# bcgsc/abyss

Hardware: NVIDIA B200
Metric: k-mers/sec (Bloom insert + unitig extend) (higher is better)
Workload: dtype u8

## Files before the change

### abyss_b200/capi.py

```python
from __future__ import annotations

import ctypes as C
import os

import numpy as np

_HERE = os.path.dirname(os.path.abspath(__file__))
LIB_PATH = os.path.join(_HERE, "lib", "libabyssb200.so")

ABB_OK, ABB_EINVAL, ABB_ENODEV, ABB_ECUDA, ABB_ENOMEM, ABB_ESTATE = 0, -1, -2, -3, -4, -5
COUNTING, BIT, CASCADING = 0, 1, 2


class AbbError(RuntimeError):
    def __init__(self, code: int, msg: str):
        super().__init__(f"libabyssb200 error {code}: {msg}")
        self.code = code


class InsertStats(C.Structure):
    _fields_ = [("kmers", C.c_uint64), ("slots", C.c_uint64), ("windows", C.c_uint64),
                ("deferred", C.c_uint64), ("launches", C.c_uint64),
                ("ms_hash", C.c_float), ("ms_insert", C.c_float), ("ms_commit", C.c_float),
                ("commit_launches", C.c_uint64), ("commit_slots", C.c_uint64), ("drains", C.c_uint64),
# ... 60 lines not shown
    "abb_filter_set_threshold": (C.c_int, [_vp, C.c_uint]),
    "abb_insert_reads": (C.c_int, [_vp, _vp, _vp, C.c_uint64, _u64p]),
    "abb_insert_reads_dev": (C.c_int, [_vp, _vp, _vp, C.c_uint64, C.c_uint64, _u64p]),
    "abb_insert_hashes": (C.c_int, [_vp, _vp, C.c_uint64]),
    "abb_contains_hashes": (C.c_int, [_vp, _vp, C.c_uint64, _vp]),
    "abb_mincount_hashes": (C.c_int, [_vp, _vp, C.c_uint64, _vp]),
    "abb_hash_reads": (C.c_int, [C.c_uint, C.c_char_p, _vp, _vp, C.c_uint64, _vp, _vp, _u64p, C.c_int]),
    "abb_hash_reads_dev": (C.c_int, [_vp, _vp, _vp, C.c_uint64, _vp, _vp, C.c_uint64, _u64p]),
    "abb_insert_h0_dev": (C.c_int, [_vp, _vp, C.c_uint64]),
    "abb_comm_unique_id": (C.c_int, [_vp]),
    "abb_comm_create": (C.c_int, [C.POINTER(_vp), C.c_int, C.c_int, _vp, C.c_int]),
    "abb_comm_destroy": (C.c_int, [_vp]),
    "abb_comm_rank": (C.c_int, [_vp]),
    "abb_comm_world": (C.c_int, [_vp]),
    "abb_insert_reads_sharded_dev": (C.c_int, [_vp, _vp, _vp, _vp, C.c_uint64, C.c_int, _u64p]),
    "abb_insert_reads_sharded": (C.c_int, [_vp, _vp, _vp, _vp, C.c_uint64, C.c_int, _u64p]),
    "abb_filter_resident_reads": (C.c_int, [_vp, C.POINTER(_vp), C.POINTER(_vp), _u64p]),
    "abb_filter_allgather": (C.c_int, [_vp, _vp]),
    "abb_comm_allgather_bytes": (C.c_int, [_vp, _vp, C.c_uint64, _vp]),
    "abb_comm_allreduce_max_u8": (C.c_int, [_vp, _vp, C.c_uint64, _vp]),
    "abb_comm_exchange_bytes": (C.c_int, [_vp, _vp, C.c_uint64, _vp, _u64p, _u64p, _vp]),
    "abb_filter_device_ptr": (_vp, [_vp, C.c_int]),
    "abb_filter_download": (C.c_int, [_vp, C.c_int, _vp, C.c_uint64]),
    "abb_filter_upload": (C.c_int, [_vp, C.c_int, _vp, C.c_uint64]),
    "abb_filter_clear": (C.c_int, [_vp]),
    "abb_filter_popcount": (C.c_int, [_vp, _u64p, _u64p]),
    "abb_assembler_create": (C.c_int, [C.POINTER(_vp), _vp, C.POINTER(AssemblyParams)]),
    "abb_assembler_destroy": (C.c_int, [_vp]),
    "abb_assembler_process_reads": (C.c_int, [_vp, _vp, _vp, C.c_uint64, C.POINTER(C.POINTER(Contig)), _u64p, C.POINTER(C.c_char_p)]),
    "abb_assembler_process_reads_dev": (C.c_int, [_vp, _vp, _vp, C.c_uint64, C.POINTER(C.POINTER(Contig)), _u64p, C.POINTER(C.c_char_p)]),
    "abb_assembler_stats": (C.c_int, [_vp, C.POINTER(AssemblyStats)]),
    "abb_assembler_reset": (C.c_int, [_vp]),
    "abb_assembler_classify_dev": (C.c_int, [_vp, _vp, _vp, C.c_uint64, _vp]),
    "abb_assembler_set_codes": (C.c_int, [_vp, _vp, C.c_uint64]),
    "abb_assembler_counters": (C.c_int, [_vp, C.POINTER(AssemblyCounters)]),
    "abb_assembler_set_counters": (C.c_int, [_vp, C.POINTER(AssemblyCounters)]),
    "abb_assembler_read_results": (C.c_int, [_vp, C.POINTER(_u8p), _u64p]),
    "abb_assembler_set_comm": (C.c_int, [_vp, _vp]),
    "abb_assembler_trace": (C.c_int, [_vp, C.POINTER(C.POINTER(TraceRow)), _u64p]),
    "abb_assembler_assembled_filter": (_vp, [_vp]),
    "abb_filter_insert_stats": (C.c_int, [_vp, C.POINTER(InsertStats), C.c_int]),
    "abb_filter_set_window": (C.c_int, [_vp, C.c_uint64]),
    "abb_filter_set_profiling": (C.c_int, [_vp, C.c_int]),
    "abb_filter_stream": (_vp, [_vp]),
    "abb_contains_reads": (C.c_int, [_vp, _vp, _vp, C.c_uint64, _vp, _vp, C.c_uint64, _u64p]),
    "abb_successors": (C.c_int, [_vp, _vp, C.c_uint64, C.c_uint, _vp, _vp, _vp]),
# ... 193 lines not shown
        h, n = self._hashes(hashes)
        out = np.zeros(n, dtype=np.uint8)
        check(self._lib.abb_contains_hashes(self._h, _ptr(h), n, _ptr(out)))
        return out.astype(bool)

    def minCount(self, hashes) -> np.ndarray:
        h, n = self._hashes(hashes)
        out = np.zeros(n, dtype=np.uint8)
        check(self._lib.abb_mincount_hashes(self._h, _ptr(h), n, _ptr(out)))
        return out

    def download(self, level: int = -1) -> np.ndarray:
        out = np.empty(self.sizeInBytes(), dtype=np.uint8)
        check(self._lib.abb_filter_download(self._h, level, _ptr(out), out.size))
        return out

    def upload(self, data: np.ndarray, level: int = -1):
        d = np.ascontiguousarray(data, dtype=np.uint8)
        check(self._lib.abb_filter_upload(self._h, level, _ptr(d), d.size))

    def clear(self):
        check(self._lib.abb_filter_clear(self._h))

    def popcounts(self) -> tuple[int, int]:
        a, b = C.c_uint64(0), C.c_uint64(0)
        check(self._lib.abb_filter_popcount(self._h, C.byref(a), C.byref(b)))
        return a.value, b.value

    def popCount(self): return self.popcounts()[0]
    def filtered_popcount(self): return self.popcounts()[1]
    def FPR(self): return (self.popCount() / self.size()) ** self.getHashNum()
    def filtered_FPR(self): return (self.filtered_popcount() / self.size()) ** self.getHashNum()

    def stats(self, reset: bool = False) -> InsertStats:
        st = InsertStats()
        check(self._lib.abb_filter_insert_stats(self._h, C.byref(st), int(reset)))
        return st


READ_CODES = ["SHORTER_THAN_K", "NON_ACGT", "BLUNT_END", "NOT_SOLID", "ALL_KMERS_VISITED", "GENERATED_CONTIGS", "CANDIDATE"]


class Assembler:

    def __init__(self, solid: Filter, trim: int | None = None, read_log: bool = False, verbose: int = 0):
        self._lib = load()
# ... 164 lines not shown
```

### abyss_b200/csrc/abb_api.cu

```cuda
#include "abb_common.h"
#include "abb_insert.cuh"
#include "abb_shard.cuh"
#include <dlfcn.h>
#include <nccl.h>
#include <cub/device/device_scan.cuh>
#include <algorithm>
#include <cstdlib>
#include <cstring>
#include <new>
#include <vector>

namespace abb {

static thread_local char g_err[512] = "";

void set_error(const char* fmt, ...)
{
	va_list ap;
	va_start(ap, fmt);
	vsnprintf(g_err, sizeof g_err, fmt, ap);
	va_end(ap);
}

constexpr uint64_t kDefaultWindow = 1ULL << 17;
// ... 18 lines not shown
	}
	if (device < 0 || device >= n) {
		set_error("device %d out of range (0..%d)", device, n - 1);
		return ABB_EINVAL;
	}
	ABB_CUDA(cudaSetDevice(device));
	static int fetch = -1;
	if (fetch < 0) {
		const char* e = getenv("ABB_L2_FETCH");
		fetch = e ? atoi(e) : 0;
	}
	if (fetch > 0)
		cudaDeviceSetLimit(cudaLimitMaxL2FetchGranularity, (size_t)fetch);
	return ABB_OK;
}

static FilterView view_of(const abb_filter* f)
{
	FilterView v;
	v.data = f->d_data;
	v.level_stride = f->bytes_per_level;
	v.levels = f->levels;
	return v;
}

static uint64_t map_entries_for(uint64_t filter_size, unsigned lg = 25)
{
	if (const char* e = getenv("ABB_MAP_LOG2")) {
		const int v = atoi(e);
		if (v >= 10 && v <= 32)
			lg = (unsigned)v;
	}
	uint64_t want = 1ULL << lg;
	const uint64_t fit = std::max<uint64_t>(next_pow2(filter_size), 1024);
	return std::min(want, fit);
}

static unsigned age_windows_for(uint64_t window)
{
	return (unsigned)std::min<uint64_t>(kMaxAgeWindows, ((1ULL << kPrioBits) - 2) / window - 1);
}

static int ensure_workspace(abb_filter* f)
{
	const uint64_t want_entries = map_entries_for(f->size, f->map_log2 ? f->map_log2 : 25);
	if (f->d_carry && f->ws_window == f->window && f->ws_H == f->H && f->map_entries == want_entries)
// ... 101 lines not shown
};

template <int KIND, bool LITERAL, int MAXH>
static int launch_windows(const InsertArgs& args, int device, cudaStream_t st)
{
	static int grid_cache[64] = { 0 };
	int& grid = grid_cache[device & 63];
	if (grid == 0) {
		int per_sm = 0, sms = 0;
		ABB_CUDA(cudaOccupancyMaxActiveBlocksPerMultiprocessor(&per_sm, k_insert_windows<KIND, LITERAL, MAXH>, 256, 0));
		ABB_CUDA(cudaDeviceGetAttribute(&sms, cudaDevAttrMultiProcessorCount, device));
		grid = std::max(1, per_sm) * sms;
	}
	void* params[] = { (void*)&args };
	ABB_CUDA(cudaLaunchCooperativeKernel((void*)k_insert_windows<KIND, LITERAL, MAXH>, dim3((unsigned)grid), dim3(256), params, 0, st));
	return ABB_OK;
}

template <bool LITERAL>
static int ordered_insert(abb_filter* f, const uint64_t* d_hashes, const uint8_t* d_valid, uint64_t n_slots)
{
	if (n_slots == 0)
		return ABB_OK;
	if (f->kind == ABB_BIT) {
		ABB_DISPATCH_H(f->H, (k_bits_insert<LITERAL, MAXH><<<blocks_for(n_slots, 256), 256, 0, f->stream>>>(
		                         d_hashes, d_valid, n_slots, f->cfg, f->d_data)));
		f->st.launches += 1;
		ABB_CUDA(cudaGetLastError());
		return ABB_OK;
	}
	ABB_CHECK(ensure_workspace(f));
	cudaStream_t st = f->stream;
	const uint64_t W = f->window;
	const uint64_t n_windows = (n_slots + W - 1) / W;
	ABB_REQUIRE(n_windows < (1ULL << 31), "too many windows in one call");
	const uint64_t cap = W + kCarryLanes;
	InsertArgs a;
	a.hashes = d_hashes;
	a.valid = d_valid;
	a.n_slots = n_slots;
	a.window = (unsigned)W;
	a.w_begin = 0;
	a.n_windows = (unsigned)n_windows;
	a.cfg = f->cfg;
	for (int i = 0; i < 3; ++i) {
		a.map[i].w = f->d_map[i];
// ... 332 lines not shown
}

struct abb_comm {
	ncclComm_t comm = nullptr;
	int rank = 0, world = 1, device = 0;
};

namespace abb {

static uint64_t shard_chunk(uint64_t size, unsigned world) { return ((size + world - 1) / world + 15) & ~15ULL; }

static uint64_t sharded_window(const abb_filter* f, unsigned world)
{
	uint64_t w = 2 * f->window * world;
	if (const char* e = getenv("ABB_SHARD_WINDOW"))
		w = strtoull(e, nullptr, 10);
	return std::min<uint64_t>(std::max<uint64_t>(w, 32), 1ULL << 21);
}

static int sharded_ordered_insert(abb_filter* f, abb_comm* c, const uint64_t* d_h0, const uint8_t* d_valid, uint64_t n_slots)
{
	if (n_slots == 0)
		return ABB_OK;
	const uint64_t user_window = f->window;
	f->window = sharded_window(f, (unsigned)c->world);
	f->map_log2 = 27;
	int rc = ensure_workspace(f);
	const uint64_t W = f->window;
	f->window = user_window;
	f->map_log2 = 0;
	ABB_CHECK(rc);
	const unsigned max_lanes = (unsigned)std::min<uint64_t>((uint64_t)kCarryLanes * (unsigned)c->world, W / 2 + kCarryLanes);
	ABB_CHECK(f->sh_buf.reserve(2 * (W + (uint64_t)max_lanes) + 64));
	cudaStream_t st = f->stream;
	const uint64_t n_windows = (n_slots + W - 1) / W;
	const unsigned age_off = (unsigned)(age_windows_for(W) * W);
	const unsigned drain_age = age_off / 3 * 2;
	const uint64_t cap = 3 * (W + kCarryLanes) / 2;
	uint64_t* carry[2] = { f->d_carry, f->d_carry + cap };
	ShardCtl* ctl = reinterpret_cast<ShardCtl*>(f->d_ctl);
	unsigned* d_nout = f->d_ctl + 4;
	const size_t map_bytes = std::max<size_t>(f->map_entries / 4, 256);
	ConflictMap maps[2] = { { f->d_map[0], f->map_entries - 1 }, { f->d_map[1], f->map_entries - 1 } };
	const uint64_t chunk = shard_chunk(f->size, (unsigned)c->world);
	Shard sh;
	sh.lo = std::min<uint64_t>(f->size, (uint64_t)c->rank * chunk);
// ... 193 lines not shown
	ABB_TRY(cudaMalloc((void**)&f->d_stats, 8 * sizeof(unsigned long long)));
	ABB_TRY(cudaMemsetAsync(f->d_stats, 0, 8 * sizeof(unsigned long long), f->stream));
	if (!f->mask.empty()) {
		std::vector<uint8_t> care(k);
		for (unsigned i = 0; i < k; ++i)
			care[i] = f->mask[i] == '1';
		ABB_TRY(cudaMalloc((void**)&f->d_care, k));
		ABB_TRY(cudaMemcpyAsync(f->d_care, care.data(), k, cudaMemcpyHostToDevice, f->stream));
	}
	ABB_TRY(cudaStreamSynchronize(f->stream));
#undef ABB_TRY
	*out = f;
	return ABB_OK;
}

int abb_filter_destroy(abb_filter* f)
{
	if (!f)
		return ABB_OK;
	cudaSetDevice(f->device);
	if (f->stream)
		cudaStreamSynchronize(f->stream);
	cudaFree(f->d_data);
	cudaFree(f->d_care);
	cudaFree(f->d_tags2[0]);
	cudaFree(f->d_tags2[1]);
	cudaFree(f->d_map[0]);
	cudaFree(f->d_carry);
	cudaFree(f->d_slotbits);
	cudaFree(f->d_ctl);
	cudaFree(f->d_stats);
	f->bases.release();
	f->offs.release();
	f->slot_offs.release();
	f->h0.release();
	f->lit.release();
	f->bounds.release();
	f->gq_kmers.release();
	f->gq_info.release();
	f->gq_len.release();
	f->gq_self.release();
	f->valid.release();
	f->scan_tmp.release();
	f->out8.release();
	f->sh_buf.release();
	for (auto e : f->prof_ev)
// ... 257 lines not shown
int abb_comm_destroy(abb_comm* c)
{
	if (!c)
		return ABB_OK;
	cudaSetDevice(c->device);
	if (c->comm && g_nccl.CommDestroy)
		g_nccl.CommDestroy(c->comm);
	delete c;
	return ABB_OK;
}

int abb_comm_rank(const abb_comm* c) { return c ? c->rank : 0; }
int abb_comm_world(const abb_comm* c) { return c ? c->world : 1; }

int abb_filter_allgather(abb_filter* f, abb_comm* c)
{
	ABB_REQUIRE(f && c, "NULL argument");
	ABB_REQUIRE(f->levels == 1, "only single-level filters are sharded");
	ABB_CUDA(cudaSetDevice(f->device));
	if (c->world == 1 || f->replicated_insert)
		return ABB_OK;
	const uint64_t chunk = shard_chunk(f->bytes_per_level, (unsigned)c->world);
	ABB_REQUIRE(chunk * c->world <= f->bytes_per_level + 4096, "too many ranks for the all-gather slack");
	ABB_NCCL(g_nccl.AllGather(f->d_data + (uint64_t)c->rank * chunk, f->d_data, chunk, ncclUint8, c->comm, f->stream));
	ABB_CUDA(cudaStreamSynchronize(f->stream));
	return ABB_OK;
}

int abb_comm_allgather_bytes(abb_comm* c, void* d_buf, uint64_t bytes_per_rank, void* cuda_stream)
{
	ABB_REQUIRE(c && (d_buf || bytes_per_rank == 0), "NULL argument");
	if (c->world == 1 || bytes_per_rank == 0)
		return ABB_OK;
	ABB_CUDA(cudaSetDevice(c->device));
	ABB_NCCL(g_nccl.AllGather((const uint8_t*)d_buf + (uint64_t)c->rank * bytes_per_rank, d_buf, bytes_per_rank, ncclUint8, c->comm,
	                          (cudaStream_t)cuda_stream));
	return ABB_OK;
}

int abb_comm_exchange_bytes(abb_comm* c, const void* d_send, uint64_t send_bytes, void* d_recv_base, const uint64_t* recv_offsets,
                            const uint64_t* recv_bytes, void* cuda_stream)
{
	ABB_REQUIRE(c && recv_offsets && recv_bytes, "NULL argument");
	if (c->world == 1)
		return ABB_OK;
	ABB_CUDA(cudaSetDevice(c->device));
// ... 27 lines not shown
	ABB_REQUIRE(f && c, "NULL argument");
	ABB_REQUIRE(f->kind == ABB_COUNTING, "the sharded insert is implemented for counting filters");
	ABB_REQUIRE(n_reads == 0 || (d_bases && d_offsets), "NULL read buffers");
	ABB_REQUIRE(f->device == c->device, "filter and communicator live on different devices");
	ABB_CUDA(cudaSetDevice(f->device));
	const bool shard = shard_policy(c->world);
	f->replicated_insert = !shard;
	ABB_CHECK(insert_reads_dev(f, (const uint8_t*)d_bases, d_offsets, n_reads, n_kmers_out, shard ? c : nullptr));
	if (finalize)
		ABB_CHECK(abb_filter_allgather(f, c));
	return ABB_OK;
}

void* abb_filter_device_ptr(abb_filter* f, int level)
{
	if (!f)
		return nullptr;
	if (level < 0)
		level = (int)f->levels - 1;
	if ((unsigned)level >= f->levels)
		return nullptr;
	cudaSetDevice(f->device);
	cudaStreamSynchronize(f->stream);
	return f->d_data + (uint64_t)level * f->bytes_per_level;
}

static int query_hashes(abb_filter* f, const uint64_t* hashes, uint64_t n, uint8_t* out, bool want_min)
{
	ABB_REQUIRE(f, "NULL filter");
	if (n == 0)
		return ABB_OK;
	ABB_REQUIRE(hashes && out, "NULL buffer");
	ABB_CUDA(cudaSetDevice(f->device));
	ABB_CHECK(f->lit.reserve(n * f->H));
	ABB_CHECK(f->out8.reserve(n));
	ABB_CUDA(cudaMemcpyAsync(f->lit.p, hashes, n * f->H * sizeof(uint64_t), cudaMemcpyHostToDevice, f->stream));
	const FilterView fv = view_of(f);
	if (f->kind == ABB_COUNTING)
		k_query<0><<<blocks_for(n, 256), 256, 0, f->stream>>>(f->lit.p, n, f->cfg, fv, f->threshold, want_min ? nullptr : f->out8.p,
		                                                       want_min ? f->out8.p : nullptr);
	else
		k_query<1><<<blocks_for(n, 256), 256, 0, f->stream>>>(f->lit.p, n, f->cfg, fv, 0, want_min ? nullptr : f->out8.p,
		                                                       want_min ? f->out8.p : nullptr);
	f->st.launches += 1;
	ABB_CUDA(cudaGetLastError());
	ABB_CUDA(cudaMemcpyAsync(out, f->out8.p, n, cudaMemcpyDeviceToHost, f->stream));
// ... 170 lines not shown
	ABB_REQUIRE(nbytes == f->bytes_per_level, "buffer is %llu bytes, the filter level is %llu", (unsigned long long)nbytes,
	            (unsigned long long)f->bytes_per_level);
	*p = f->d_data + (uint64_t)level * f->bytes_per_level;
	return ABB_OK;
}

int abb_filter_download(abb_filter* f, int level, uint8_t* host, uint64_t nbytes)
{
	uint8_t* p = nullptr;
	ABB_CHECK(level_ptr(f, level, nbytes, &p));
	ABB_REQUIRE(host, "NULL buffer");
	ABB_CUDA(cudaSetDevice(f->device));
	ABB_CUDA(cudaMemcpyAsync(host, p, nbytes, cudaMemcpyDeviceToHost, f->stream));
	ABB_CUDA(cudaStreamSynchronize(f->stream));
	return ABB_OK;
}

int abb_filter_upload(abb_filter* f, int level, const uint8_t* host, uint64_t nbytes)
{
	uint8_t* p = nullptr;
	ABB_CHECK(level_ptr(f, level, nbytes, &p));
	ABB_REQUIRE(host, "NULL buffer");
	ABB_CUDA(cudaSetDevice(f->device));
	ABB_CUDA(cudaMemcpyAsync(p, host, nbytes, cudaMemcpyHostToDevice, f->stream));
	ABB_CUDA(cudaStreamSynchronize(f->stream));
	return ABB_OK;
}

int abb_filter_clear(abb_filter* f)
{
	ABB_REQUIRE(f, "NULL filter");
	ABB_CUDA(cudaSetDevice(f->device));
	ABB_CUDA(cudaMemsetAsync(f->d_data, 0, f->bytes_per_level * f->levels, f->stream));
	ABB_CUDA(cudaStreamSynchronize(f->stream));
	return ABB_OK;
}

int abb_filter_popcount(abb_filter* f, uint64_t* nonzero, uint64_t* at_or_above_threshold)
{
	ABB_REQUIRE(f, "NULL filter");
	ABB_CUDA(cudaSetDevice(f->device));
	ABB_CUDA(cudaMemsetAsync(f->d_stats + 4, 0, 2 * sizeof(unsigned long long), f->stream));
	const uint8_t* p = f->d_data + (uint64_t)(f->levels - 1) * f->bytes_per_level;
	k_popcount<<<148 * 8, 256, 0, f->stream>>>(p, f->bytes_per_level, f->kind == ABB_COUNTING, f->threshold, f->d_stats + 4);
	f->st.launches += 1;
	ABB_CUDA(cudaGetLastError());
	unsigned long long h[2] = { 0, 0 };
	ABB_CUDA(cudaMemcpyAsync(h, f->d_stats + 4, sizeof h, cudaMemcpyDeviceToHost, f->stream));
	ABB_CUDA(cudaStreamSynchronize(f->stream));
	if (nonzero)
		*nonzero = h[0];
	if (at_or_above_threshold)
		*at_or_above_threshold = f->kind == ABB_COUNTING ? h[1] : h[0];
	return ABB_OK;
}

// ... 24 lines not shown
```

### abyss_b200/csrc/abb_assemble.cu

```cuda
#include "abb_common.h"
#include "abb_walk.cuh"
#include <cooperative_groups.h>
#include <cub/device/device_select.cuh>
#include <thrust/iterator/counting_iterator.h>
#include <algorithm>
#include <chrono>
#include <cstdlib>
#include <cstring>
#include <new>
#include <vector>

namespace abb {
namespace cg = cooperative_groups;

__host__ __device__ inline uint64_t tile_slot(uint64_t key, unsigned cls, unsigned mask)
{
	return (((key ^ (0x9E3779B97F4A7C15ULL * (cls + 1))) * 0xD6E8FEB86659FD93ULL) >> 24) & mask;
}

struct WarpCtx {
	unsigned k, trim;
	RollTab rt;
	const HashCfg* cfg;
	const uint8_t* counters;
	unsigned threshold;
	unsigned lane;
	Frame* frames;
	uint64_t* look;
	uint8_t* arena;
	unsigned long long arena_size;
	unsigned long long* arena_top;
	unsigned fail_;
	const TileRec* tile_recs;
	const unsigned* tile_tab;
	unsigned tile_mask;

	unsigned long long* dbg = nullptr;
	long long t_last = 0;
	__device__ void tick(int slot)
	{
		if (!dbg)
			return;
		const long long now = clock64();
		if (slot >= 0 && lane == 0)
			dbg[slot] += (unsigned long long)(now - t_last);
		t_last = now;
	}
	__device__ bool tiles_enabled() const { return tile_tab != nullptr; }
// ... 5 lines not shown
				return nullptr;
			const TileRec* t = tile_recs + (v - 1);
			if (t->key == key && t->cls == cls)
				return t;
		}
	}
	__device__ uint32_t tile_index(const TileRec* t) const { return (uint32_t)(t - tile_recs); }
	__device__ const TileRec* tile_at(uint32_t idx) const { return tile_recs + idx; }
	__device__ void prefetch(const void* p) const
	{
		if (p)
			asm volatile("prefetch.global.L2 [%0];" ::"l"(p));
	}
	__device__ void wr32(uint32_t* p, uint32_t v) const { *(volatile uint32_t*)p = v; }

	struct Probe {
		bool ok;
	};
	template <int KW>
	__device__ Probe neighbors_issue(const Vtx<KW>& v) const
	{
		const unsigned n = lane >> 2, hs = lane & 3;
		const uint64_t h0 = neighbor_bloom(v, k, rt, n < 4 ? FWD : REV, n & 3);
		unsigned mn = 255;
		for (unsigned i = hs; i < cfg->H; i += 4)
			mn = min(mn, (unsigned)__ldcg(counters + nth_pos(h0, *cfg, i)));
		Probe p;
		p.ok = mn >= threshold;
		return p;
	}
	__device__ unsigned neighbors_finish(const Probe& p) const
	{
		unsigned b = __ballot_sync(0xffffffffu, p.ok);
		b &= b >> 1;
		b &= b >> 2;
		unsigned r = 0;
#pragma unroll
		for (int j = 0; j < 8; ++j)
			r |= ((b >> (4 * j)) & 1u) << j;
		return r;
	}
	template <int KW>
	__device__ unsigned neighbors(const Vtx<KW>& v) const
	{
		return neighbors_finish(neighbors_issue(v));
	}
	template <int KW>
	__device__ unsigned neighbors_dir(const Vtx<KW>& v, Dir d) const
	{
		const unsigned n = lane >> 2, hs = lane & 3;
		const bool mine = (n < 4) == (d == FWD);
		bool ok = true;
		if (mine) {
			const uint64_t h0 = neighbor_bloom(v, k, rt, n < 4 ? FWD : REV, n & 3);
			unsigned mn = 255;
			for (unsigned i = hs; i < cfg->H; i += 4)
				mn = min(mn, (unsigned)__ldcg(counters + nth_pos(h0, *cfg, i)));
			ok = mn >= threshold;
		}
		Probe p;
		p.ok = ok;
		const unsigned m = neighbors_finish(p);
		return d == FWD ? (m & 15) : (m >> 4);
	}
	__device__ uint64_t rd64(const uint64_t* p) const { return *(const volatile uint64_t*)p; }
	__device__ void wr64(uint64_t* p, uint64_t v) const { *(volatile uint64_t*)p = v; }
	__device__ uint8_t rd8(const uint8_t* p) const { return *(const volatile uint8_t*)p; }
	__device__ void wr8(uint8_t* p, uint8_t v) const { *(volatile uint8_t*)p = v; }
	__device__ void sync() const { __syncwarp(); }
	__device__ bool find64(const uint64_t* a, unsigned n, uint64_t key, unsigned stride) const
	{
		for (unsigned base = 0; base < n; base += 32) {
			const unsigned i = base + lane;
			const bool hit = i < n && *(const volatile uint64_t*)(a + (size_t)i * stride) == key;
			if (__any_sync(0xffffffffu, hit))
				return true;
		}
		return false;
	}
	__device__ uint8_t* alloc(unsigned long long bytes, bool zero)
	{
// ... 242 lines not shown
				r.seed_pos = seed_pos;
				r.psize = o.psize;
				r.left = (unsigned char)o.left;
				r.right = (unsigned char)o.right;
				r.flags = (unsigned char)((o.pushed_front ? 1 : 0) | (o.pushed_back ? 2 : 0) | (o.popped_front ? 4 : 0) | (o.popped_back ? 8 : 0));
				r.pad1 = 0;
				r.front_h = o.front_h;
				r.back_h = o.back_h;
				r.left_n = o.left_n;
				r.right_n = o.right_n;
				recs[idx] = r;
			}
		}
		++ordinal;
	}
};

struct IsCandidate {
	const uint8_t* codes;
	__host__ __device__ bool operator()(unsigned r) const { return codes[r] == RC_CANDIDATE; }
};

struct WalkCfg {
	unsigned k, trim, threshold;
	RollTab rt;
	const uint8_t* counters;
};

struct TileView {
	const TileRec* recs;
	const unsigned* tab;
	unsigned mask;
};

__device__ __forceinline__ WarpCtx make_ctx(const WalkCfg& w, const HashCfg* cfg, Frame* frames, uint64_t* look, unsigned gwarp,
                                            uint8_t* arena, unsigned long long arena_size, unsigned long long* arena_top)
{
	WarpCtx c;
	c.k = w.k;
	c.trim = w.trim;
	c.rt = w.rt;
	c.cfg = cfg;
	c.counters = w.counters;
	c.threshold = w.threshold;
	c.lane = threadIdx.x & 31;
	c.frames = frames ? frames + (size_t)gwarp * kFrameCap : nullptr;
	c.look = look + (size_t)gwarp * kLookCap;
	c.arena = arena;
	c.arena_size = arena_size;
	c.arena_top = arena_top;
	c.fail_ = 0;
	c.tile_recs = nullptr;
	c.tile_tab = nullptr;
	c.tile_mask = 0;
	return c;
}

constexpr int kWalkWarps = 4;

template <int KW>
__global__ void __launch_bounds__(kWalkWarps * 32)
k_classify(const uint8_t* __restrict__ bases, const uint64_t* __restrict__ offs, const uint64_t* __restrict__ slot_offs,
           const uint64_t* __restrict__ h0, const uint8_t* __restrict__ valid, uint64_t n_reads, WalkCfg w,
           const __grid_constant__ HashCfg cfg, uint64_t* look, int exact_codes, uint8_t* __restrict__ codes)
{
	const unsigned gwarp = blockIdx.x * kWalkWarps + (threadIdx.x >> 5);
	const unsigned nwarps = gridDim.x * kWalkWarps;
// ... 5 lines not shown
		uint8_t code;
		if (L < w.k) {
			code = RC_SHORTER_THAN_K;
		} else {
			const uint64_t s0 = slot_offs[r];
			const unsigned nk = L - w.k + 1;
			bool bad = false;
			if (w.rt.nmask) {
				for (unsigned j = lane; j < L; j += 32)
					bad |= base_code(bases[beg + j]) >= 4;
			} else
				for (unsigned j = lane; j < nk; j += 32)
					bad |= valid[s0 + j] == 0;
			if (__any_sync(0xffffffffu, bad)) {
				code = RC_NON_ACGT;
			} else {
				bool solid = true;
				for (unsigned base = 0; base < nk && solid; base += 32) {
					const unsigned j = base + lane;
					bool ok = true;
					if (j < nk) {
						const uint64_t h = h0[s0 + j];
						for (unsigned i = 0; i < cfg.H; ++i)
							ok &= __ldcg(w.counters + nth_pos(h, cfg, i)) >= w.threshold;
					}
					solid = __all_sync(0xffffffffu, ok);
				}
				if (!solid && !exact_codes) {
					code = RC_NOT_SOLID;
				} else {
					const Vtx<KW> first = vtx_from_codes<KW>(bases + beg, w.k, true, w.rt);
					bool blunt = !look_ahead(c, first, REV, kFpTrim);
					if (!blunt) {
						const Vtx<KW> last = vtx_from_codes<KW>(bases + beg + L - w.k, w.k, true, w.rt);
						blunt = !look_ahead(c, vtx_revcomp(last, w.k), REV, kFpTrim);
					}
					code = blunt ? RC_BLUNT_END : (solid ? RC_CANDIDATE : RC_NOT_SOLID);
				}
			}
		}
		if (lane == 0)
			codes[r] = code;
	}
}

__global__ void __launch_bounds__(256)
k_visited(const unsigned* __restrict__ cand, unsigned c0, unsigned n, const uint64_t* __restrict__ slot_offs,
// ... 42 lines not shown
	const uint64_t beg = offs[r];
	const unsigned L = (unsigned)(offs[r + 1] - beg);
	DevEmit emit = { recs, nrecs, rec_cap, gwarp, 0 };
	const bool ok = walk_read<KW>(c, bases + beg, L, emit);
	if (c.lane == 0)
		status[gwarp] = ok ? 0u : (c.fail_ ? c.fail_ : 1u);
}


__global__ void __launch_bounds__(256)
k_find_markers(const uint64_t* __restrict__ h0, const uint8_t* __restrict__ valid, const uint64_t* __restrict__ slot_offs,
               uint64_t n_reads, uint64_t n_slots, WalkCfg w, const __grid_constant__ HashCfg cfg, unsigned long long* mset,
               unsigned mset_mask, unsigned long long* __restrict__ out , unsigned* n_out,
               unsigned out_cap, unsigned world, unsigned rank)
{
	for (uint64_t s = (uint64_t)blockIdx.x * blockDim.x + threadIdx.x; s < n_slots; s += (uint64_t)gridDim.x * blockDim.x) {
		const uint64_t h = h0[s];
		if (!is_marker(h) || !valid[s])
			continue;
		if (world > 1 && (unsigned)((h >> 8) % world) != rank)
			continue;
		bool solid = true;
		for (unsigned i = 0; i < cfg.H; ++i)
			solid &= __ldcg(w.counters + nth_pos(h, cfg, i)) >= w.threshold;
		if (!solid)
			continue;
		const unsigned long long key = h ? h : 1;
		bool fresh = false;
		for (uint64_t t = pathset_slot(key, mset_mask + 1);; t = (t + 1) & mset_mask) {
			const unsigned long long old = atomicCAS(mset + t, 0ULL, key);
			if (old == 0ULL) {
				fresh = true;
				break;
			}
			if (old == key)
				break;
		}
		if (!fresh)
			continue;
		uint64_t lo = 0, hi = n_reads;
		while (lo < hi) {
			const uint64_t mid = (lo + hi) / 2;
			if (slot_offs[mid + 1] <= s)
				lo = mid + 1;
			else
				hi = mid;
		}
// ... 475 lines not shown
	}
}

}

using namespace abb;

struct abb_assembler {
	abb_filter* solid = nullptr;
	abb_filter* assembled = nullptr;
	abb_assembly_params params = {};
	abb_assembly_counters counters = {};
	cudaStream_t stream = nullptr;
	uint64_t reads_seen = 0;
	int kw = 0;
	RollTab rt;
	uint8_t* d_mpos = nullptr;
	const uint8_t* ext_codes = nullptr;
	uint64_t ext_n = 0;
	abb_comm* comm = nullptr;
	DevBuf<uint8_t> gather;
	const uint8_t* cur_bases = nullptr;
	const uint64_t* cur_offs = nullptr;

	DevBuf<uint8_t> bases, valid, codes, vis, scan_tmp, cseq, cvalid, rcode, caccept;
	DevBuf<uint64_t> offs, slot_offs, h0, coffs, cslot, ch0;
	DevBuf<unsigned> cand, spec, spec_cbeg, clen, ccov, status, seg_contig, seg_len, big_idx, big_spec;
	DevBuf<uint64_t> seg_beg, seg_slot, rep_off;
	DevBuf<ContigRec> recs, recs_sorted;
	DevBuf<Frame> frames;
	DevBuf<uint64_t> look;
	unsigned scratch_warps = 0;
	uint8_t* d_arena = nullptr;
	unsigned long long arena_size = 0;
	unsigned long long* d_arena_top = nullptr;
	unsigned* d_nrecs = nullptr;
	unsigned long long* d_ends = nullptr;
	unsigned ends_cap = 0;
	unsigned* d_ends_n = nullptr;
	uint64_t ends_upper = 0;

	bool tiles_on = true;
	TileRec* d_tiles = nullptr;
	unsigned tile_cap = 0;
	unsigned* d_tile_tab = nullptr;
	unsigned tile_tab_mask = 0;
// ... 74 lines not shown
	uint64_t ncap = a->ends_cap ? a->ends_cap : 1024;
	while (ncap < need)
		ncap <<= 1;
	ABB_REQUIRE(ncap <= (1ULL << 31), "contigEndKmers table too large");
	unsigned long long* nt = nullptr;
	ABB_CUDA(cudaMalloc((void**)&nt, ncap * sizeof(unsigned long long)));
	ABB_CUDA(cudaMemsetAsync(nt, 0, ncap * sizeof(unsigned long long), a->stream));
	if (a->d_ends) {
		k_endset_rehash<<<256, 256, 0, a->stream>>>(a->d_ends, a->ends_cap, nt, (unsigned)ncap);
		ABB_CUDA(cudaGetLastError());
		ABB_CUDA(cudaStreamSynchronize(a->stream));
		cudaFree(a->d_ends);
	}
	a->d_ends = nt;
	a->ends_cap = (unsigned)ncap;
	return ABB_OK;
}

WalkCfg walk_cfg(const abb_assembler* a)
{
	WalkCfg w;
	w.k = a->solid->k;
	w.trim = a->params.trim;
	w.threshold = a->solid->threshold;
	w.rt = a->rt;
	w.counters = a->solid->d_data;
	return w;
}

#define ABB_DISPATCH_KW(kw, ...)              \
	do {                                      \
		switch (kw) {                         \
		case 1: { constexpr int KW = 1; __VA_ARGS__; } break; \
		case 2: { constexpr int KW = 2; __VA_ARGS__; } break; \
		case 3: { constexpr int KW = 3; __VA_ARGS__; } break; \
		case 4: { constexpr int KW = 4; __VA_ARGS__; } break; \
		default: { constexpr int KW = 6; __VA_ARGS__; } break; \
		}                                     \
	} while (0)

template <typename T>
int h2d(DevBuf<T>& d, const std::vector<T>& h, cudaStream_t s)
{
	ABB_CHECK(d.reserve(h.size() + 1));
	if (!h.empty())
		ABB_CUDA(cudaMemcpyAsync(d.p, h.data(), h.size() * sizeof(T), cudaMemcpyHostToDevice, s));
	return ABB_OK;
}

// ... 747 lines not shown
	cudaFree(a->d_ends_n);
	if (a->ev[0]) cudaEventDestroy(a->ev[0]);
	if (a->ev[1]) cudaEventDestroy(a->ev[1]);
	if (a->ev2[0]) cudaEventDestroy(a->ev2[0]);
	if (a->ev2[1]) cudaEventDestroy(a->ev2[1]);
	delete a;
	return ABB_OK;
}

static int hash_and_classify(abb_assembler* a, const uint8_t* d_bases, const uint64_t* d_offs, uint64_t n_reads, bool classify,
                             uint64_t* total_out)
{
	abb_filter* f = a->solid;
	cudaStream_t st = a->stream;
	uint64_t total = 0;
	ABB_CHECK(compute_slot_offsets(f->k, d_offs, n_reads, a->slot_offs, a->scan_tmp, st, &total, &a->st_launches));
	ABB_CHECK(a->h0.reserve(total + 1));
	ABB_CHECK(a->valid.reserve(total + 1));
	ABB_CHECK(a->codes.reserve(n_reads));
	if (total)
		ABB_CHECK(launch_hash(nullptr, f->k, f->d_care, d_bases, d_offs, a->slot_offs.p, 0, n_reads, 0, a->h0.p, a->valid.p, st,
		                      &a->st_launches));
	*total_out = total;
	if (!classify)
		return ABB_OK;
	int sms = 148;
	cudaDeviceGetAttribute(&sms, cudaDevAttrMultiProcessorCount, f->device);
	const unsigned world = a->comm ? (unsigned)abb_comm_world(a->comm) : 1u, rank = a->comm ? (unsigned)abb_comm_rank(a->comm) : 0u;
	const uint64_t lo = rank * n_reads / world, up = (rank + 1) * n_reads / world;
	const unsigned grid = (unsigned)std::min<uint64_t>(blocks_for(std::max<uint64_t>(up - lo, 1), kWalkWarps), (uint64_t)sms * 8);
	ABB_CHECK(ensure_scratch(a, grid * kWalkWarps));
	const WalkCfg w = walk_cfg(a);
	if (up > lo)
		ABB_DISPATCH_KW(a->kw, (k_classify<KW><<<grid, kWalkWarps * 32, 0, st>>>(d_bases, d_offs + lo, a->slot_offs.p + lo, a->h0.p, a->valid.p,
		                                                                        up - lo, w, f->cfg, a->look.p, (int)a->params.read_log,
		                                                                        a->codes.p + lo)));
	ABB_CUDA(cudaGetLastError());
	++a->st_launches;
	if (world > 1)
		ABB_CHECK(allgather_slices(a, a->codes.p + lo, n_reads, a->codes.p));
	return ABB_OK;
}

static int process_batch(abb_assembler* a, const uint8_t* d_bases, const uint64_t* d_offs, uint64_t n_reads,
                         const abb_contig** contigs, uint64_t* n_contigs, const char** seqs)
{
// ... 225 lines not shown
```

### abyss_b200/csrc/abb_common.h

```cpp
#pragma once
#include "../../include/abyss_b200.h"
#include "abb_device.cuh"
#include <cuda_runtime.h>
#include <cstdarg>
#include <cstdio>
#include <string>
#include <vector>

namespace abb {

void set_error(const char* fmt, ...);

#define ABB_CUDA(call)                                                                             \
	do {                                                                                           \
		cudaError_t e__ = (call);                                                                  \
		if (e__ != cudaSuccess) {                                                                  \
			abb::set_error("%s:%d: %s failed: %s", __FILE__, __LINE__, #call, cudaGetErrorString(e__)); \
			return (e__ == cudaErrorMemoryAllocation) ? ABB_ENOMEM                                 \
			       : (e__ == cudaErrorNoDevice || e__ == cudaErrorInsufficientDriver) ? ABB_ENODEV \
			                                                                          : ABB_ECUDA; \
		}                                                                                          \
	} while (0)

#define ABB_CHECK(expr)            \
// ... 79 lines not shown
	uint64_t tag_slots = 0;
	uint64_t* d_carry = nullptr;
	unsigned* d_slotbits = nullptr;
	uint64_t slotbit_words = 0;
	unsigned* d_ctl = nullptr;
	unsigned long long* d_stats = nullptr;

	uint64_t resident_reads = 0;
	bool l2_policy_held = false;
	bool replicated_insert = false;
	abb::DevBuf<uint8_t> bases;
	abb::DevBuf<uint64_t> offs, slot_offs, h0, lit, bounds;
	abb::DevBuf<uint8_t> valid, scan_tmp, out8, sh_buf;
	abb::DevBuf<uint8_t> gq_kmers;
	abb::DevBuf<abb_succ_info> gq_info;
	abb::DevBuf<unsigned> gq_len;
	abb::DevBuf<uint64_t> gq_self;

	abb_insert_stats st = {};
	bool profile = false;
	uint64_t prof_stride = 1, prof_slots = 0, sh_drains = 0;
	std::vector<cudaEvent_t> prof_ev;
	size_t prof_used = 0;
};
```

### abyss_b200/csrc/abb_insert.cuh

```cuda
#pragma once
#include "abb_device.cuh"
#include "abb_graph.cuh"
#include <cooperative_groups.h>
#include <cuda/barrier>
#include <cuda_runtime.h>

namespace abb {
namespace cg = cooperative_groups;

constexpr unsigned kPrioBits = 28;
constexpr unsigned kMaxAgeWindows = 48;
constexpr unsigned kCarryLanes = 1u << 16;
constexpr unsigned kPosBits = 36;
constexpr uint64_t kPrioMask = (1ULL << kPrioBits) - 1;

struct TagTable {
	unsigned long long* e;
	uint64_t mask;
};

ABB_D uint64_t tag_pack(uint64_t pos, uint64_t prio) { return ((pos + 1) << kPrioBits) | prio; }
ABB_D uint64_t tag_home(uint64_t pos, const TagTable& t)
{
	return ((pos * 0x9E3779B97F4A7C15ULL) >> 20) & t.mask;
// ... 890 lines not shown
			} else
				nz += __popc(x[j]);
		}
	}
	if (blockIdx.x == 0 && threadIdx.x == 0)
		for (uint64_t i = nwords * 16; i < nbytes; ++i) {
			unsigned c = data[i];
			if (counting) {
				nz += c != 0;
				th += c >= threshold;
			} else
				nz += __popc(c);
		}
	for (int d = 16; d; d >>= 1) {
		nz += __shfl_down_sync(0xffffffffu, nz, d);
		th += __shfl_down_sync(0xffffffffu, th, d);
	}
	if ((threadIdx.x & 31) == 0) {
		atomicAdd(&out[0], nz);
		atomicAdd(&out[1], th);
	}
}

}
```

### include/abyss_b200.h

```cpp
#ifndef ABYSS_B200_H
#define ABYSS_B200_H

#include <stddef.h>
#include <stdint.h>

#ifdef __cplusplus
extern "C" {
#endif

#define ABB_VERSION 100

enum {
	ABB_OK = 0,
	ABB_EINVAL = -1,
	ABB_ENODEV = -2,
	ABB_ECUDA = -3,
	ABB_ENOMEM = -4,
	ABB_ESTATE = -5
};

enum {
	ABB_COUNTING = 0,
	ABB_BIT = 1,
	ABB_CASCADING = 2
// ... 36 lines not shown

typedef struct abb_comm abb_comm;
int abb_comm_unique_id(uint8_t id_out[128]);
int abb_comm_create(abb_comm** out, int rank, int world, const uint8_t id[128], int device);
int abb_comm_destroy(abb_comm* c);
int abb_comm_rank(const abb_comm* c);
int abb_comm_world(const abb_comm* c);
int abb_insert_reads_sharded_dev(abb_filter* f, abb_comm* c, const char* d_bases, const uint64_t* d_offsets, uint64_t n_reads,
                                 int finalize, uint64_t* n_kmers_out);
int abb_insert_reads_sharded(abb_filter* f, abb_comm* c, const char* bases, const uint64_t* offsets, uint64_t n_reads, int finalize,
                             uint64_t* n_kmers_out);
int abb_filter_allgather(abb_filter* f, abb_comm* c);
int abb_filter_resident_reads(abb_filter* f, const char** d_bases, const uint64_t** d_offsets, uint64_t* n_reads);
int abb_comm_allgather_bytes(abb_comm* c, void* d_buf, uint64_t bytes_per_rank, void* cuda_stream);
int abb_comm_allreduce_max_u8(abb_comm* c, void* d_buf, uint64_t n, void* cuda_stream);
int abb_comm_exchange_bytes(abb_comm* c, const void* d_send, uint64_t send_bytes, void* d_recv_base, const uint64_t* recv_offsets,
                            const uint64_t* recv_bytes, void* cuda_stream);

void* abb_filter_device_ptr(abb_filter* f, int level);

int abb_filter_download(abb_filter* f, int level, uint8_t* host, uint64_t nbytes);
int abb_filter_upload(abb_filter* f, int level, const uint8_t* host, uint64_t nbytes);
int abb_filter_clear(abb_filter* f);

int abb_filter_popcount(abb_filter* f, uint64_t* nonzero, uint64_t* at_or_above_threshold);

typedef struct abb_assembly_params {
	unsigned trim;
	unsigned verbose;
	unsigned read_log;
	unsigned reserved;
} abb_assembly_params;

typedef struct abb_contig {
	uint64_t seed_read;
	uint64_t seq_offset;
	uint32_t length;
	uint32_t coverage;
} abb_contig;

typedef struct abb_assembly_counters {
	uint64_t solid_reads, visited_reads, reads_processed, bases_assembled, contig_id;
} abb_assembly_counters;

int abb_assembler_create(abb_assembler** out, abb_filter* solid, const abb_assembly_params* params);
int abb_assembler_destroy(abb_assembler* a);
// ... 89 lines not shown
```

Before: 993.5 million.

## Compress counting filter into solid bitmap for unitig extension probes

Before extension, the byte-per-slot counting filter is converted into a 1-bit-per-slot solid bitmap (count >= threshold), cached by a version counter and rebuilt when the filter changes or raw pointers are exposed. All solidity probes in the walk, neighbor and tile kernels read this bitmap instead of comparing counter bytes. The aim is an 8x smaller probe working set that fits better in L2, cutting random-access memory traffic. It costs an extra full pass over the filter per process call when invalidated, and adds version tracking that external raw writes may bypass.

```diff
diff --git a/abyss_b200/capi.py b/abyss_b200/capi.py
--- a/abyss_b200/capi.py
+++ b/abyss_b200/capi.py
@@ -106,6 +106,7 @@
     "abb_comm_exchange_bytes": (C.c_int, [_vp, _vp, C.c_uint64, _vp, _u64p, _u64p, _vp]),
     "abb_filter_device_ptr": (_vp, [_vp, C.c_int]),
     "abb_filter_download": (C.c_int, [_vp, C.c_int, _vp, C.c_uint64]),
+    "abb_filter_download_solid": (C.c_int, [_vp, _vp, C.c_uint64]),
     "abb_filter_upload": (C.c_int, [_vp, C.c_int, _vp, C.c_uint64]),
     "abb_filter_clear": (C.c_int, [_vp]),
     "abb_filter_popcount": (C.c_int, [_vp, _u64p, _u64p]),
@@ -345,6 +346,11 @@
     def clear(self):
         check(self._lib.abb_filter_clear(self._h))
 
+    def download_solid(self) -> np.ndarray:
+        out = np.empty((self.size() + 7) // 8, dtype=np.uint8)
+        check(self._lib.abb_filter_download_solid(self._h, _ptr(out), out.size))
+        return out
+
     def popcounts(self) -> tuple[int, int]:
         a, b = C.c_uint64(0), C.c_uint64(0)
         check(self._lib.abb_filter_popcount(self._h, C.byref(a), C.byref(b)))
diff --git a/abyss_b200/csrc/abb_api.cu b/abyss_b200/csrc/abb_api.cu
--- a/abyss_b200/csrc/abb_api.cu
+++ b/abyss_b200/csrc/abb_api.cu
@@ -64,6 +64,25 @@
 	v.level_stride = f->bytes_per_level;
 	v.levels = f->levels;
 	return v;
+}
+
+int solid_bitmap(abb_filter* f, cudaStream_t st, const uint8_t** bits)
+{
+	ABB_REQUIRE(f && f->kind == ABB_COUNTING, "the solid bitmap needs a counting filter");
+	ABB_CUDA(cudaSetDevice(f->device));
+	const uint64_t nwords = (f->size + 31) / 32;
+	if (!f->d_solid) {
+		ABB_CUDA(cudaMalloc((void**)&f->d_solid, nwords * 4 + 16));
+		f->solid_version = 0;
+	}
+	if (f->raw_exposed || f->solid_version != f->version || f->solid_threshold != f->threshold) {
+		k_solid_bits<<<148 * 8, 256, 0, st>>>(f->d_data, f->size, f->threshold, (uint32_t*)f->d_solid);
+		ABB_CUDA(cudaGetLastError());
+		f->solid_version = f->version;
+		f->solid_threshold = f->threshold;
+	}
+	*bits = f->d_solid;
+	return ABB_OK;
 }
 
 static uint64_t map_entries_for(uint64_t filter_size, unsigned lg = 25)
@@ -211,6 +230,7 @@
 {
 	if (n_slots == 0)
 		return ABB_OK;
+	++f->version;
 	if (f->kind == ABB_BIT) {
 		ABB_DISPATCH_H(f->H, (k_bits_insert<LITERAL, MAXH><<<blocks_for(n_slots, 256), 256, 0, f->stream>>>(
 		                         d_hashes, d_valid, n_slots, f->cfg, f->d_data)));
@@ -589,6 +609,7 @@
 {
 	if (n_slots == 0)
 		return ABB_OK;
+	++f->version;
 	const uint64_t user_window = f->window;
 	f->window = sharded_window(f, (unsigned)c->world);
 	f->map_log2 = 27;
@@ -828,6 +849,7 @@
 	if (f->stream)
 		cudaStreamSynchronize(f->stream);
 	cudaFree(f->d_data);
+	cudaFree(f->d_solid);
 	cudaFree(f->d_care);
 	cudaFree(f->d_tags2[0]);
 	cudaFree(f->d_tags2[1]);
@@ -1131,6 +1153,7 @@
 		return ABB_OK;
 	const uint64_t chunk = shard_chunk(f->bytes_per_level, (unsigned)c->world);
 	ABB_REQUIRE(chunk * c->world <= f->bytes_per_level + 4096, "too many ranks for the all-gather slack");
+	++f->version;
 	ABB_NCCL(g_nccl.AllGather(f->d_data + (uint64_t)c->rank * chunk, f->d_data, chunk, ncclUint8, c->comm, f->stream));
 	ABB_CUDA(cudaStreamSynchronize(f->stream));
 	return ABB_OK;
@@ -1204,6 +1227,7 @@
 		return nullptr;
 	cudaSetDevice(f->device);
 	cudaStreamSynchronize(f->stream);
+	f->raw_exposed = true;
 	return f->d_data + (uint64_t)level * f->bytes_per_level;
 }
 
@@ -1420,6 +1444,7 @@
 	ABB_CHECK(level_ptr(f, level, nbytes, &p));
 	ABB_REQUIRE(host, "NULL buffer");
 	ABB_CUDA(cudaSetDevice(f->device));
+	++f->version;
 	ABB_CUDA(cudaMemcpyAsync(p, host, nbytes, cudaMemcpyHostToDevice, f->stream));
 	ABB_CUDA(cudaStreamSynchronize(f->stream));
 	return ABB_OK;
@@ -1428,8 +1453,22 @@
 int abb_filter_clear(abb_filter* f)
 {
 	ABB_REQUIRE(f, "NULL filter");
+	++f->version;
 	ABB_CUDA(cudaSetDevice(f->device));
 	ABB_CUDA(cudaMemsetAsync(f->d_data, 0, f->bytes_per_level * f->levels, f->stream));
+	ABB_CUDA(cudaStreamSynchronize(f->stream));
+	return ABB_OK;
+}
+
+int abb_filter_download_solid(abb_filter* f, uint8_t* host, uint64_t nbytes)
+{
+	ABB_REQUIRE(f && host, "NULL argument");
+	ABB_REQUIRE(f->kind == ABB_COUNTING, "the solid bitmap needs a counting filter");
+	ABB_REQUIRE(nbytes == (f->size + 7) / 8, "buffer is %llu bytes, the solid bitmap is %llu", (unsigned long long)nbytes,
+	            (unsigned long long)((f->size + 7) / 8));
+	const uint8_t* bits = nullptr;
+	ABB_CHECK(solid_bitmap(f, f->stream, &bits));
+	ABB_CUDA(cudaMemcpyAsync(host, bits, nbytes, cudaMemcpyDeviceToHost, f->stream));
 	ABB_CUDA(cudaStreamSynchronize(f->stream));
 	return ABB_OK;
 }
diff --git a/abyss_b200/csrc/abb_assemble.cu b/abyss_b200/csrc/abb_assemble.cu
--- a/abyss_b200/csrc/abb_assemble.cu
+++ b/abyss_b200/csrc/abb_assemble.cu
@@ -18,12 +18,13 @@
 	return (((key ^ (0x9E3779B97F4A7C15ULL * (cls + 1))) * 0xD6E8FEB86659FD93ULL) >> 24) & mask;
 }
 
+__device__ __forceinline__ bool solid_bit(const uint8_t* bits, uint64_t p) { return (__ldcg(bits + (p >> 3)) >> (p & 7)) & 1; }
+
 struct WarpCtx {
 	unsigned k, trim;
 	RollTab rt;
 	const HashCfg* cfg;
-	const uint8_t* counters;
-	unsigned threshold;
+	const uint8_t* solid;
 	unsigned lane;
 	Frame* frames;
 	uint64_t* look;
@@ -75,11 +76,11 @@
 	{
 		const unsigned n = lane >> 2, hs = lane & 3;
 		const uint64_t h0 = neighbor_bloom(v, k, rt, n < 4 ? FWD : REV, n & 3);
-		unsigned mn = 255;
+		bool ok = true;
 		for (unsigned i = hs; i < cfg->H; i += 4)
-			mn = min(mn, (unsigned)__ldcg(counters + nth_pos(h0, *cfg, i)));
+			ok &= solid_bit(solid, nth_pos(h0, *cfg, i));
 		Probe p;
-		p.ok = mn >= threshold;
+		p.ok = ok;
 		return p;
 	}
 	__device__ unsigned neighbors_finish(const Probe& p) const
@@ -106,10 +107,8 @@
 		bool ok = true;
 		if (mine) {
 			const uint64_t h0 = neighbor_bloom(v, k, rt, n < 4 ? FWD : REV, n & 3);
-			unsigned mn = 255;
 			for (unsigned i = hs; i < cfg->H; i += 4)
-				mn = min(mn, (unsigned)__ldcg(counters + nth_pos(h0, *cfg, i)));
-			ok = mn >= threshold;
+				ok &= solid_bit(solid, nth_pos(h0, *cfg, i));
 		}
 		Probe p;
 		p.ok = ok;
@@ -398,9 +397,9 @@
 };
 
 struct WalkCfg {
-	unsigned k, trim, threshold;
+	unsigned k, trim;
 	RollTab rt;
-	const uint8_t* counters;
+	const uint8_t* solid;
 };
 
 struct TileView {
@@ -417,8 +416,7 @@
 	c.trim = w.trim;
 	c.rt = w.rt;
 	c.cfg = cfg;
-	c.counters = w.counters;
-	c.threshold = w.threshold;
+	c.solid = w.solid;
 	c.lane = threadIdx.x & 31;
 	c.frames = frames ? frames + (size_t)gwarp * kFrameCap : nullptr;
 	c.look = look + (size_t)gwarp * kLookCap;
@@ -470,7 +468,7 @@
 					if (j < nk) {
 						const uint64_t h = h0[s0 + j];
 						for (unsigned i = 0; i < cfg.H; ++i)
-							ok &= __ldcg(w.counters + nth_pos(h, cfg, i)) >= w.threshold;
+							ok &= solid_bit(w.solid, nth_pos(h, cfg, i));
 					}
 					solid = __all_sync(0xffffffffu, ok);
 				}
@@ -559,7 +557,7 @@
 			continue;
 		bool solid = true;
 		for (unsigned i = 0; i < cfg.H; ++i)
-			solid &= __ldcg(w.counters + nth_pos(h, cfg, i)) >= w.threshold;
+			solid &= solid_bit(w.solid, nth_pos(h, cfg, i));
 		if (!solid)
 			continue;
 		const unsigned long long key = h ? h : 1;
@@ -1081,6 +1079,7 @@
 	DevBuf<uint8_t> gather;
 	const uint8_t* cur_bases = nullptr;
 	const uint64_t* cur_offs = nullptr;
+	const uint8_t* solid_bits = nullptr;
 
 	DevBuf<uint8_t> bases, valid, codes, vis, scan_tmp, cseq, cvalid, rcode, caccept;
 	DevBuf<uint64_t> offs, slot_offs, h0, coffs, cslot, ch0;
@@ -1201,9 +1200,8 @@
 	WalkCfg w;
 	w.k = a->solid->k;
 	w.trim = a->params.trim;
-	w.threshold = a->solid->threshold;
 	w.rt = a->rt;
-	w.counters = a->solid->d_data;
+	w.solid = a->solid_bits;
 	return w;
 }
 
@@ -1997,6 +1995,7 @@
 		ABB_CHECK(launch_hash(nullptr, f->k, f->d_care, d_bases, d_offs, a->slot_offs.p, 0, n_reads, 0, a->h0.p, a->valid.p, st,
 		                      &a->st_launches));
 	*total_out = total;
+	ABB_CHECK(solid_bitmap(f, st, &a->solid_bits));
 	if (!classify)
 		return ABB_OK;
 	int sms = 148;
diff --git a/abyss_b200/csrc/abb_common.h b/abyss_b200/csrc/abb_common.h
--- a/abyss_b200/csrc/abb_common.h
+++ b/abyss_b200/csrc/abb_common.h
@@ -125,4 +125,14 @@
 	uint64_t prof_stride = 1, prof_slots = 0, sh_drains = 0;
 	std::vector<cudaEvent_t> prof_ev;
 	size_t prof_used = 0;
+
+	uint64_t version = 1;
+	bool raw_exposed = false;
+	uint8_t* d_solid = nullptr;
+	uint64_t solid_version = 0;
+	unsigned solid_threshold = 0;
 };
+
+namespace abb {
+int solid_bitmap(abb_filter* f, cudaStream_t st, const uint8_t** bits);
+}
diff --git a/abyss_b200/csrc/abb_insert.cuh b/abyss_b200/csrc/abb_insert.cuh
--- a/abyss_b200/csrc/abb_insert.cuh
+++ b/abyss_b200/csrc/abb_insert.cuh
@@ -936,4 +936,27 @@
 	}
 }
 
-}
+static __global__ void __launch_bounds__(256)
+k_solid_bits(const uint8_t* __restrict__ counters, uint64_t n, unsigned threshold, uint32_t* __restrict__ bits)
+{
+	const uint64_t nwords = (n + 31) / 32;
+	const unsigned t4 = min(threshold, 255u) * 0x01010101u;
+	for (uint64_t i = (uint64_t)blockIdx.x * blockDim.x + threadIdx.x; i < nwords; i += (uint64_t)gridDim.x * blockDim.x) {
+		const uint4* src = reinterpret_cast<const uint4*>(counters + 32 * i);
+		const uint4 a = __ldcs(src), b = __ldcs(src + 1);
+		const unsigned x[8] = { a.x, a.y, a.z, a.w, b.x, b.y, b.z, b.w };
+		uint32_t w = 0;
+#pragma unroll
+		for (int j = 0; j < 8; ++j) {
+			const unsigned m = __vcmpgeu4(x[j], t4) & 0x01010101u;
+			w |= (((m * 0x01020408u) >> 24) & 15u) << (4 * j);
+		}
+		if (threshold > 255)
+			w = 0;
+		if (32 * i + 32 > n)
+			w &= (1u << (unsigned)(n - 32 * i)) - 1u;
+		bits[i] = w;
+	}
+}
+
+}
diff --git a/include/abyss_b200.h b/include/abyss_b200.h
--- a/include/abyss_b200.h
+++ b/include/abyss_b200.h
@@ -82,6 +82,7 @@
 int abb_filter_download(abb_filter* f, int level, uint8_t* host, uint64_t nbytes);
 int abb_filter_upload(abb_filter* f, int level, const uint8_t* host, uint64_t nbytes);
 int abb_filter_clear(abb_filter* f);
+int abb_filter_download_solid(abb_filter* f, uint8_t* host, uint64_t nbytes);
 
 int abb_filter_popcount(abb_filter* f, uint64_t* nonzero, uint64_t* at_or_above_threshold);
 
```

Result: no change. 1.002 billion, median of 6 (+0.8%).
